# DocF/multispectral-object-detection

Hardware: AMD Instinct MI355X
Metric: image-pairs/sec fwd, yolov5l+CFTx3 640×640 bs64, 1/2/4/8 GPU (higher is better)
Workload: dtype bf16; 1 GPU; cfg3 (yolov5l_fusion_transformerx3_FLIR_aligned) two-stream forward, 640x640, 64 pairs/GPU, BN folded, pre-NMS detections; pairs_per_gpu=64, image_size=640, parallelism=batch-shard x1, hip_graph=True, two_hip_streams=False, forwards_in_flight=3, streams_per_forward_in_flight=1, single_in_flight_streams=2

## Files before the change

### include/cft_hip.h

```cpp
#ifndef CFT_HIP_H
#define CFT_HIP_H

#ifdef __cplusplus
extern "C" {
#endif

#define CFT_ABI_VERSION 19

enum { CFT_BF16 = 0, CFT_F32 = 1, CFT_F16 = 2 };
enum { CFT_ACT_NONE = 0, CFT_ACT_SILU = 1, CFT_ACT_GELU = 2 };
enum {
  CFT_OK = 0,
  CFT_EINVAL = -1,
  CFT_ELAUNCH = -2,
  CFT_ENODEV = -3
};

int cft_abi_version(void);
int cft_device_check(void);
const char* cft_last_error(void);
int cft_clock_probe(void* out4_u64, int spin_us, int* wall_khz, void* stream);

int cft_conv2d(const void* x, const void* w, const float* bias, const void* res, void* y,
               int B, int H, int W, int cin, int ldx, int xoff,
               int n, int kpad, int ksize, int stride,
               int ldy, int yoff, int ldr, int roff,
               int act, int dtype, int out_dtype, int res_dtype, void* stream);

int cft_conv2d_chain(const void* x, const void* w1, const float* bias1, const void* w2, const float* bias2, void* y,
                     int B, int H, int W, int cin, int ldx, int xoff,
                     int n1, int kpad1, int ksize, int stride, int n2,
                     int ldy, int yoff, int act2, int dtype, void* stream);
int cft_conv2d_chain_ok(int B, int H, int W, int cin, int ldx, int n1, int kpad1, int ksize, int stride, int n2, int ldy, int dtype);

int cft_conv2d_chain_res(const void* x, const void* w1, const float* bias1, const void* res, void* y1,
                         const void* w2, const float* bias2, void* y2,
                         int B, int H, int W, int cin, int ldx, int xoff,
                         int n1, int kpad1, int ksize, int stride, int ldr, int roff, int ldy1, int yoff1,
                         int n2, int ldy2, int yoff2, int act2, int dtype, void* stream);

int cft_linear_splitk(const void* x, const void* w, const float* bias, float* parts,
                      int rows, int cin, int ldx, int n, int kpad, int splits, int dtype, void* stream);

int cft_bottleneck(const void* x, int ldx, int xoff, const void* w1, int kpad1, const float* b1,
                   const void* w2, int kpad2, const void* w2_stages, const float* b2, void* y, int ldy, int yoff,
                   int B, int H, int W, int c, int shortcut, int dtype, void* stream);

int cft_bottleneck_pack_w2(const void* w2, int kpad2, int c, void* w2_stages, int dtype, void* stream);

int cft_set_conv_variant(int variant);

int cft_focus_s2d(const float* in, void* out, int B, int H, int W, int dtype, void* stream);

int cft_focus_s2d_u8(const unsigned char* in, long stride_b, long stride_c, long stride_h, void* out,
                     int B, int H, int W, float scale, int dtype, void* stream);

int cft_focus_conv(const void* in, int in_kind, long stride_b, long stride_c, long stride_h, float scale,
                   const void* w, int kpad, const float* bias, void* y, int ldy, int yoff,
                   int B, int H, int W, int n, int act, int dtype, void* stream);

int cft_spp_maxpool(void* buf, int B, int H, int W, int C, int ld, int k1, int k2, int k3,
                    int dtype, void* stream);

int cft_copy_channels(const void* in, int ldi, int ioff, void* out, int ldo, int ooff,
                      int B, int Ho, int Wo, int C, int up, int dtype, void* stream);

int cft_to_nhwc(const void* in, int in_dtype, long stride_b, long stride_c, long stride_h, long stride_w,
                void* out, int ldo, int ooff, int B, int C, int cpad, int H, int W, int dtype, void* stream);

int cft_letterbox_u8(const unsigned char* src, int src_h, int src_w, long src_row_stride,
                     unsigned char* dst, int dst_h, int dst_w, long dst_stride_y, long dst_stride_x, long dst_stride_c, int flip_channels,
                     int resized_h, int resized_w, int top, int left, int color0, int color1, int color2, void* stream);

enum { CFT_PAIR_COPY = 0, CFT_PAIR_LINEAR = 1, CFT_PAIR_AREA = 2 };
#define CFT_PAIR_DESC_BYTES 64
#define CFT_PAIR_MAX_REDUCTION 4
typedef struct {
  const unsigned char* src_rgb;
  const unsigned char* src_ir;
  long stride_rgb, stride_ir;
  int h0, w0;
  int h, w;
  int top, left;
  int mode, flip;
} cft_pair_desc_t;
int cft_pair_batch_u8(const void* desc_dev, const void* desc_host, int B, unsigned char* dst, int dst_h, int dst_w, int color, void* stream);

enum { CFT_AUG_FLIPLR = 1, CFT_AUG_FLIPUD = 2 };
#define CFT_AUG_DESC_BYTES 400
#define CFT_AUG_TILE_BYTES 80
#define CFT_AUG_MAX_SIDE 16384
typedef struct {
  const unsigned char* src_rgb;
  const unsigned char* src_ir;
  long stride_rgb, stride_ir;
  int h0, w0;
  int h, w;
  int x1, y1, x2, y2;
  int padw, padh;
  int reserved[2];
} cft_aug_tile_t;
// ... 155 lines not shown
```

### multispectral-object-detection_amd/csrc/bneck_common.h

```cpp
#pragma once
#include "cft_common.h"

struct Bneck128Params {
  const unsigned char* x;
  const unsigned char* w1;
  const unsigned char* w2;
  const unsigned char* w2s;
  const float* b1;
  const float* b2;
  unsigned char* y;
  int ldx, xoff, ldy, yoff, kpad1, kpad2;
  int H, W, tiles_x, tiles_y, ntiles, shortcut;
};

int bneck128_asm_launch(const Bneck128Params& p, int dtype, hipStream_t stream);
```

### multispectral-object-detection_amd/csrc/bottleneck.hip

```cpp
#include "cft_common.h"
#include <stdlib.h>

#ifdef CFT_PROBES
extern thread_local int g_conv_variant;
#endif

__device__ __attribute__((aligned(16))) uint32_t cft_zero_page_b[4] = {0u, 0u, 0u, 0u};
typedef __attribute__((address_space(3))) void lds_void_t;
typedef const __attribute__((address_space(1))) void gbl_void_t;

#include "bneck_common.h"

template <typename T, int ABL = 0>
__global__ void __launch_bounds__(512, 4) bottleneck128c_kernel(const Bneck128Params p) {
  constexpr int C = 128, TH = 8, TW = 16, PW = TW + 2, PH = TH + 2, NPIX = PW * PH;
  constexpr int NRT = (NPIX + 15) / 16;
  constexpr int PLANE = NRT * 16 * 128;
  constexpr int SLOT = 8192;
  constexpr int SLD = 64 + 4;
  constexpr int RW = 2;
  constexpr int XS = (ABL & 4) ? 0 : 2 * RW;
  static_assert(PW == 18 && NRT == 12, "the mul-shift below divides by 18; 8 + 4 row tiles");
  extern __shared__ __attribute__((aligned(16))) unsigned char smem[];
  unsigned char* sT = smem;
// ... 206 lines not shown
#undef BNC_MMA
#undef BNC_FETCH_RS

    if constexpr (ABL & 4) {
#pragma unroll
      for (int i = 0; i < RW; ++i)
#pragma unroll
        for (int j = 0; j < 4; ++j) asm volatile("" ::"v"(acc[i][j]));
    } else {
      float b2v[4];
#pragma unroll
      for (int j = 0; j < 4; ++j) b2v[j] = sB[C + wnc * 64 + j * 16 + lrow];
      asm volatile("s_waitcnt lgkmcnt(0)" ::: "memory");
      __builtin_amdgcn_s_barrier();
      float* stage = reinterpret_cast<float*>(sT) + wave * (16 * SLD);
#pragma unroll
      for (int i = 0; i < RW; ++i) {
#pragma unroll
        for (int j = 0; j < 4; ++j)
#pragma unroll
          for (int e = 0; e < 4; ++e)
            stage[(lgrp * 4 + e) * SLD + j * 16 + lrow] = apply_act<(ABL & 512) ? CFT_ACT_NONE : CFT_ACT_SILU>(acc[i][j][e] + b2v[j]);
        __builtin_amdgcn_fence(__ATOMIC_RELEASE, "wavefront");
        __builtin_amdgcn_wave_barrier();
        __builtin_amdgcn_fence(__ATOMIC_ACQUIRE, "wavefront");
#pragma unroll
        for (int v = 0; v < 2; ++v) {
          const int it = lane + v * 64;
          const int row = it >> 3, col = (it & 7) * 8;
          const int x = x0 + row, y = y0 + wmr * RW + i;
          if (x < p.W && y < p.H) {
            const f32x4_t s0 = *reinterpret_cast<const f32x4_t*>(stage + row * SLD + col);
            const f32x4_t s1 = *reinterpret_cast<const f32x4_t*>(stage + row * SLD + col + 4);
            float o[8] = {s0[0], s0[1], s0[2], s0[3], s1[0], s1[1], s1[2], s1[3]};
            if (p.shortcut) {
              float rf[8];
              Elem<T>::unpack(rs[i][v], rf);
#pragma unroll
              for (int e = 0; e < 8; ++e) o[e] += rf[e];
            }
            *reinterpret_cast<gran_t*>(p.y + ((img_pix + (long)y * p.W + x) * p.ldy + p.yoff + wnc * 64 + col) * 2) = Elem<T>::pack(o);
          }
        }
        __builtin_amdgcn_fence(__ATOMIC_RELEASE, "wavefront");
        __builtin_amdgcn_wave_barrier();
        __builtin_amdgcn_fence(__ATOMIC_ACQUIRE, "wavefront");
      }
    }
  }
#undef BNC_STAGE
#undef BNC_SYNC
}

template <typename T, int ABL = 0>
__global__ void __launch_bounds__(512, 4) bottleneck64r_kernel(const Bneck128Params p) {
  constexpr int C = 64, TS = 16, PW = TS + 2, NPIX = PW * PW;
  constexpr int NRT = (NPIX + 15) / 16;
  constexpr int PATCH = NRT * 16 * 128;
  constexpr int SLOT = 8192;
  constexpr int SLD = 64 + 4;
  constexpr int RW = 2, RT1 = 3;
  static_assert(PW == 18, "the mul-shift below divides by 18");
  extern __shared__ __attribute__((aligned(16))) unsigned char smem[];
  unsigned char* sT = smem;
  unsigned char* sR = smem + PATCH;
  float* sB = reinterpret_cast<float*>(smem + NPIX * 128);

  const int tid = threadIdx.x, lane = tid & 63;
  const int wave = __builtin_amdgcn_readfirstlane(tid >> 6);
  const int lrow = lane & 15, lgrp = lane >> 4;
  const int tiles = p.tiles_x * p.tiles_y;
  const int nb_ = gridDim.x, bid_ = blockIdx.x;
  const int xq_ = nb_ >> 3, xr_ = nb_ & 7, xcd_ = bid_ & 7, xslot_ = bid_ >> 3;
  const int ltile = (xcd_ < xr_ ? xcd_ * (xq_ + 1) : xr_ * (xq_ + 1) + (xcd_ - xr_) * xq_) + xslot_;
  const int b = ltile / tiles, tt = ltile - b * tiles;
  const int ty = tt / p.tiles_x, tx = tt - ty * p.tiles_x;
  const int y0 = ty * TS, x0 = tx * TS;
  const long img_pix = (long)b * p.H * p.W;
  const uint32_t tl = (uint32_t)(uintptr_t)(lds_void_t*)sT;

  const int r1 = tid >> 3, g1 = (tid & 7) ^ (r1 & 7);
  const unsigned char* src1 = p.w1 + ((long)r1 * p.kpad1 + g1 * 8) * 2;
  const unsigned char* src2 = p.w2 + ((long)r1 * p.kpad2 + g1 * 8) * 2;
#define BNR_STAGE(s_)                                                                                    \
  {                                                                                                      \
    const int ss_ = (s_);                                                                                \
    const unsigned char* src_ = ss_ == 0 ? src1 : src2 + (long)(ss_ - 1) * 128;                          \
    if constexpr (!(ABL & 8))                                                                            \
      __builtin_amdgcn_global_load_lds((gbl_void_t*)src_, (lds_void_t*)(sR + (ss_ & 3) * SLOT + wave * 1024), 16, 0, 0); \
  }
#define BNR_SYNC(n_)                                                                                     \
  {                                                                                                      \
    __builtin_amdgcn_sched_barrier(0);                                                                   \
    __builtin_amdgcn_s_waitcnt((n_) | 0x70);                                    \
    __builtin_amdgcn_s_barrier();                                                                        \
    __builtin_amdgcn_sched_barrier(0);                                                                   \
  }
  const int fb = lrow * 128 + ((lgrp ^ (lrow & 7)) << 4);

  gran_t a1[RT1][2];
  uint32_t keep[RT1];
#pragma unroll
  for (int it = 0; it < RT1; ++it) {
    const int q = (wave + 8 * it) * 16 + lrow;
    const int py = (q * 3641) >> 16, px = q - py * PW;
    const int zy = min(max(y0 - 1 + py, 0), p.H - 1), zx = min(max(x0 - 1 + px, 0), p.W - 1);
    keep[it] = (q < NPIX && (unsigned)(y0 - 1 + py) < (unsigned)p.H && (unsigned)(x0 - 1 + px) < (unsigned)p.W) ? 0xffffffffu : 0u;
    const unsigned char* xp = p.x + ((img_pix + (long)zy * p.W + zx) * p.ldx + p.xoff + lgrp * 8) * 2;
#pragma unroll
    for (int ks = 0; ks < 2; ++ks) {
      gran_t t = {0u, 0u, 0u, 0u};
      if (wave + 8 * it < NRT) t = *reinterpret_cast<const gran_t*>(xp + ks * 64);
      a1[it][ks] = t;
    }
  }
  __builtin_amdgcn_sched_barrier(0);
  BNR_STAGE(0)
  BNR_STAGE(1)
  BNR_STAGE(2)
  __builtin_amdgcn_sched_barrier(0);
  {
    float bq = 0.0f;
    if (tid < C) { if (p.b1 != nullptr) bq = p.b1[tid]; }
    else if (tid < 2 * C) { if (p.b2 != nullptr) bq = p.b2[tid - C]; }
    if (tid < 2 * C) sB[tid] = bq;
  }
  BNR_SYNC(0)
#pragma unroll
  for (int it = 0; it < RT1; ++it)
#pragma unroll
    for (int ks = 0; ks < 2; ++ks) {
      a1[it][ks].x &= keep[it]; a1[it][ks].y &= keep[it]; a1[it][ks].z &= keep[it]; a1[it][ks].w &= keep[it];
    }

  {
    f32x4_t acc1[RT1][4];
#pragma unroll
    for (int it = 0; it < RT1; ++it)
#pragma unroll
      for (int j = 0; j < 4; ++j) acc1[it][j] = f32x4_t{0.f, 0.f, 0.f, 0.f};
    BNR_STAGE(3)
    gran_t wf[4][2];
#pragma unroll
    for (int j = 0; j < 4; ++j) {
      wf[j][0] = *reinterpret_cast<const gran_t*>(sR + j * 2048 + fb);
      wf[j][1] = *reinterpret_cast<const gran_t*>(sR + j * 2048 + (fb ^ 64));
    }
    if constexpr (!(ABL & 1)) {
#pragma unroll
      for (int it = 0; it < RT1; ++it)
        if (wave + 8 * it < NRT) {
#pragma unroll
          for (int ks = 0; ks < 2; ++ks)
#pragma unroll
            for (int j = 0; j < 4; ++j) acc1[it][j] = mma_granule<T>(wf[j][ks], a1[it][ks], acc1[it][j]);
        }
    }
    BNR_SYNC(2)
#pragma unroll
    for (int it = 0; it < RT1; ++it) {
      const int q = (wave + 8 * it) * 16 + lrow;
      if (wave + 8 * it < NRT && q < NPIX) {
#pragma unroll
        for (int j = 0; j < 4; ++j) {
          const int cc = j * 16 + lgrp * 4;
          const f32x4_t b1q = *reinterpret_cast<const f32x4_t*>(sB + cc);
          float v[4];
#pragma unroll
          for (int e = 0; e < 4; ++e) v[e] = (ABL & 1) ? 0.0f : apply_act<CFT_ACT_SILU>(acc1[it][j][e] + b1q[e]);
          uint2 w;
          w.x = Elem<T>::pack2(v[0], v[1]) & keep[it];
          w.y = Elem<T>::pack2(v[2], v[3]) & keep[it];
          const uint32_t ta = tl + q * 128 + ((((cc >> 3) ^ (q & 7)) << 4) | ((cc & 7) << 1));
          const unsigned long long wq = ((unsigned long long)w.y << 32) | w.x;
          asm volatile("ds_write_b64 %0, %1" ::"v"(ta), "v"(wq) : "memory");
        }
      }
// ... 12 lines not shown
  for (int i = 0; i < RW; ++i) af[1][i] = gran_t{0u, 0u, 0u, 0u};
#pragma unroll
  for (int j = 0; j < 4; ++j) bf[1][j] = gran_t{0u, 0u, 0u, 0u};
#define BNR_READ(slot_, ks_)                                                                             \
  {                                                                                                      \
    _Pragma("unroll") for (int i = 0; i < RW; ++i) {                                                     \
      const int q = qb + i * PW;                                                                         \
      af[ks_][i] = *reinterpret_cast<const gran_t*>(sT + q * 128 + ((((ks_) * 4 + lgrp) ^ (q & 7)) << 4)); \
    }                                                                                                    \
    _Pragma("unroll") for (int j = 0; j < 4; ++j)                                                        \
      bf[ks_][j] = *reinterpret_cast<const gran_t*>(sR + (slot_) * SLOT + j * 2048 + ((ks_) ? (fb ^ 64) : fb)); \
    __builtin_amdgcn_sched_barrier(0);                                                                   \
  }
#define BNR_MMA(set_)                                                                                    \
  {                                                                                                      \
    _Pragma("unroll") for (int i = 0; i < RW; ++i)                                                       \
      _Pragma("unroll") for (int j = 0; j < 4; ++j) {                                                    \
        if constexpr (ABL & 2) { asm volatile("" ::"v"(af[set_][i]), "v"(bf[set_][j])); }                \
        else acc[i][j] = mma_granule<T>(af[set_][i], bf[set_][j], acc[i][j]);                            \
      }                                                                                                  \
    __builtin_amdgcn_sched_barrier(0);                                                                   \
  }
#pragma unroll
  for (int tap = 0; tap < 9; ++tap) {
    const int kh = tap / 3, kw = tap - kh * 3;
    const int qb = (wave * RW + kh) * PW + kw + lrow;
    if (tap + 4 <= 9) BNR_STAGE(tap + 4)
    BNR_READ((1 + tap) & 3, 0)
    BNR_MMA(1)
    BNR_READ((1 + tap) & 3, 1)
    BNR_MMA(0)
    if (tap <= 5) { BNR_SYNC(2) }
    else if (tap == 6) { BNR_SYNC(1) }
    else if (tap == 7) { BNR_SYNC(0) }
  }
  BNR_MMA(1)
#undef BNR_READ
#undef BNR_MMA
#undef BNR_STAGE
#undef BNR_SYNC

  if constexpr (ABL & 4) {
#pragma unroll
    for (int i = 0; i < RW; ++i)
#pragma unroll
      for (int j = 0; j < 4; ++j) asm volatile("" ::"v"(acc[i][j]));
    return;
  }
  float b2v[4];
#pragma unroll
  for (int j = 0; j < 4; ++j) b2v[j] = sB[C + j * 16 + lrow];
  asm volatile("s_waitcnt lgkmcnt(0)" ::: "memory");
  __builtin_amdgcn_s_barrier();
  if (p.shortcut) {
    int lane_e;
    asm volatile("v_mbcnt_lo_u32_b32 %0, -1, 0\n\tv_mbcnt_hi_u32_b32 %0, -1, %0" : "=v"(lane_e));
    const int lrow_e = lane_e & 15, lgrp_e = lane_e >> 4;
#pragma unroll
    for (int it = 0; it < RT1; ++it) {
      const int q = (wave + 8 * it) * 16 + lrow_e;
      const int py = (q * 3641) >> 16, px = q - py * PW;
      if (wave + 8 * it < NRT && py >= 1 && py <= TS && px >= 1 && px <= TS) {
        const int c = (py - 1) * TS + (px - 1);
#pragma unroll
        for (int ks = 0; ks < 2; ++ks)
          *reinterpret_cast<gran_t*>(sR + c * 128 + (((ks * 4 + lgrp_e) ^ (c & 7)) << 4)) = a1[it][ks];
      }
    }
    asm volatile("s_waitcnt lgkmcnt(0)" ::: "memory");
    __builtin_amdgcn_s_barrier();
  }
  float* stage = reinterpret_cast<float*>(sT) + wave * (16 * SLD);
#pragma unroll
  for (int i = 0; i < RW; ++i) {
#pragma unroll
    for (int j = 0; j < 4; ++j)
#pragma unroll
      for (int e = 0; e < 4; ++e)
        stage[(lgrp * 4 + e) * SLD + j * 16 + lrow] = apply_act<CFT_ACT_SILU>(acc[i][j][e] + b2v[j]);
    __builtin_amdgcn_fence(__ATOMIC_RELEASE, "wavefront");
    __builtin_amdgcn_wave_barrier();
    __builtin_amdgcn_fence(__ATOMIC_ACQUIRE, "wavefront");
#pragma unroll
    for (int v = 0; v < 2; ++v) {
      const int it = lane + v * 64;
      const int row = it >> 3, col = (it & 7) * 8;
      const int x = x0 + row, y = y0 + wave * RW + i;
      if (x < p.W && y < p.H) {
        const f32x4_t s0 = *reinterpret_cast<const f32x4_t*>(stage + row * SLD + col);
        const f32x4_t s1 = *reinterpret_cast<const f32x4_t*>(stage + row * SLD + col + 4);
        float o[8] = {s0[0], s0[1], s0[2], s0[3], s1[0], s1[1], s1[2], s1[3]};
        if (p.shortcut) {
          const int c = (wave * RW + i) * TS + row;
          const gran_t rsv = *reinterpret_cast<const gran_t*>(sR + c * 128 + (((it & 7) ^ (c & 7)) << 4));
          float rf[8];
          Elem<T>::unpack(rsv, rf);
#pragma unroll
          for (int e = 0; e < 8; ++e) o[e] += rf[e];
        }
        *reinterpret_cast<gran_t*>(p.y + ((img_pix + (long)y * p.W + x) * p.ldy + p.yoff + col) * 2) = Elem<T>::pack(o);
      }
    }
    __builtin_amdgcn_fence(__ATOMIC_RELEASE, "wavefront");
    __builtin_amdgcn_wave_barrier();
    __builtin_amdgcn_fence(__ATOMIC_ACQUIRE, "wavefront");
  }
}

__global__ void __launch_bounds__(256) bneck_pack_w2_kernel(const gran_t* __restrict__ w2, int kpad2, gran_t* __restrict__ out, int total) {
  const int i = blockIdx.x * 256 + threadIdx.x;
  if (i >= total) return;
  const int slot = i & 3, n = (i >> 2) & 127, u = i >> 9;
  const int kg = slot ^ ((0x1320 >> (4 * ((n >> 2) & 3))) & 3);
  out[i] = w2[(long)n * (kpad2 / 8) + u * 4 + kg];
}

extern "C" int cft_bottleneck_pack_w2(const void* w2, int kpad2, int c, void* w2_stages, int dtype, void* stream) {
  CFT_REQUIRE(w2 && w2_stages, "cft_bottleneck_pack_w2: null pointer");
  CFT_REQUIRE(dtype == CFT_BF16 || dtype == CFT_F16, "cft_bottleneck_pack_w2: dtype must be CFT_BF16 or CFT_F16");
  CFT_REQUIRE(c == 128 && kpad2 == 9 * 128, "cft_bottleneck_pack_w2: 128 channels, kpad2 = 1152");
  const int total = 36 * 128 * 4;
  hipLaunchKernelGGL(bneck_pack_w2_kernel, dim3((total + 255) / 256), dim3(256), 0, as_stream(stream),
                     (const gran_t*)w2, kpad2, (gran_t*)w2_stages, total);
// ... 27 lines not shown
  q.b1 = b1; q.b2 = b2; q.y = (unsigned char*)y;
  q.ldx = ldx; q.xoff = xoff; q.ldy = ldy; q.yoff = yoff; q.kpad1 = kpad1; q.kpad2 = kpad2;
  q.H = H; q.W = W; q.shortcut = shortcut ? 1 : 0;
  q.tiles_x = (W + 15) / 16; q.tiles_y = c == 128 ? (H + 7) / 8 : (H + 15) / 16;
  CFT_REQUIRE((long)B * q.tiles_x * q.tiles_y < (1L << 31), "cft_bottleneck: too many tiles");
  q.ntiles = B * q.tiles_x * q.tiles_y;
  hipStream_t s_ = as_stream(stream);
  const dim3 grid(q.ntiles);
#define BNC_LAUNCH(T_, ABL_)                                                                          \
  {                                                                                                   \
    constexpr int smem_ = 2 * 12 * 16 * 128 + 2 * 16384;                                              \
    cft_allow_lds<&bottleneck128c_kernel<T_, ABL_>>(smem_);                                           \
    hipLaunchKernelGGL((bottleneck128c_kernel<T_, ABL_>), grid, dim3(512), smem_, s_, q);             \
  }
#define BNR_LAUNCH(T_, ABL_)                                                                          \
  {                                                                                                   \
    constexpr int smem_ = 21 * 16 * 128 + 4 * 8192;                                                   \
    cft_allow_lds<&bottleneck64r_kernel<T_, ABL_>>(smem_);                                            \
    hipLaunchKernelGGL((bottleneck64r_kernel<T_, ABL_>), grid, dim3(512), smem_, s_, q);              \
  }
#ifdef CFT_PROBES
  if (dtype == CFT_BF16) {
    switch (g_conv_variant) {
      case 9201: if (c == 128) { BNC_LAUNCH(uint16_t, 1) return cft_check_launch("bottleneck128c_kernel(probe)"); } break;
      case 9202: if (c == 128) { BNC_LAUNCH(uint16_t, 2) return cft_check_launch("bottleneck128c_kernel(probe)"); } break;
      case 9204: if (c == 128) { BNC_LAUNCH(uint16_t, 4) return cft_check_launch("bottleneck128c_kernel(probe)"); } break;
      case 9208: if (c == 128) { BNC_LAUNCH(uint16_t, 8) return cft_check_launch("bottleneck128c_kernel(probe)"); } break;
      case 9456: if (c == 128) { BNC_LAUNCH(uint16_t, 256) return cft_check_launch("bottleneck128c_kernel(probe)"); } break;
      case 9712: if (c == 128) { BNC_LAUNCH(uint16_t, 512) return cft_check_launch("bottleneck128c_kernel(probe)"); } break;
      case 9601: if (c == 64) { BNR_LAUNCH(uint16_t, 1) return cft_check_launch("bottleneck64r_kernel(probe)"); } break;
      case 9602: if (c == 64) { BNR_LAUNCH(uint16_t, 2) return cft_check_launch("bottleneck64r_kernel(probe)"); } break;
      case 9604: if (c == 64) { BNR_LAUNCH(uint16_t, 4) return cft_check_launch("bottleneck64r_kernel(probe)"); } break;
      case 9608: if (c == 64) { BNR_LAUNCH(uint16_t, 8) return cft_check_launch("bottleneck64r_kernel(probe)"); } break;
      default: break;
    }
  }
#endif
  if (c == 128) {
#ifdef CFT_PROBES
    if (g_conv_variant == 98 || (g_conv_variant >= 9300 && g_conv_variant < 9400)) {
      q.tiles_y = (H + 15) / 16;
      q.ntiles = B * q.tiles_x * q.tiles_y;
      return bneck128_asm_launch(q, dtype, s_);
    }
#endif
    if (dtype == CFT_F16) BNC_LAUNCH(f16_t, 0) else BNC_LAUNCH(uint16_t, 0)
    return cft_check_launch("bottleneck128c_kernel");
  }
  if (dtype == CFT_F16) BNR_LAUNCH(f16_t, 0) else BNR_LAUNCH(uint16_t, 0)
#undef BNC_LAUNCH
#undef BNR_LAUNCH
  return cft_check_launch("bottleneck64r_kernel");
}
```

### multispectral-object-detection_amd/models/common.py

```python
import math
from collections import namedtuple

import torch
import torch.nn as nn

from .. import ops
from ..ops import ACT_GELU, ACT_NONE, ACT_SILU

BN_EPS = 1e-3


def autopad(k, p=None):
    if p is None:
        p = k // 2 if isinstance(k, int) else [x // 2 for x in k]
    return p


class _Pending:

    def materialize(self):
        raise NotImplementedError


class PendingBilinear(_Pending):
# ... 4 lines not shown
    def materialize(self, base=None):
        return ops.gpt_upsample_add(self.tokens, self.s, base, self.H, self.W, self.dtype, grid=self.grid)

    @property
    def shape(self):
        return torch.Size((self.tokens.shape[0], self.tokens.shape[2], self.H, self.W))


class PendingUpsample(_Pending):

    def __init__(self, x, up):
        self.x, self.up = x, up

    def materialize(self):
        B, C, H, W = self.x.shape
        out = ops.new_nhwc(B, H << self.up, W << self.up, C, self.x.dtype, self.x.device)
        return ops.copy_channels(self.x, out, self.up)

    @property
    def shape(self):
        B, C, H, W = self.x.shape
        return torch.Size((B, C, H << self.up, W << self.up))


class PendingConv(_Pending):

    def __init__(self, conv, x):
        self.conv, self.x = conv, x

    def materialize(self):
        return self.conv(self.x)

    @property
    def shape(self):
        B, _, H, W = self.x.shape
        return torch.Size((B, self.conv.conv.out_channels, *ops.conv_out_size(H, W, self.conv.conv.kernel_size[0], self.conv.conv.stride[0])))


def resolve(x):
    return x.materialize() if isinstance(x, _Pending) else x


def _cache_key(module, dtype, device):
    vers = tuple((int(p.data_ptr()), int(p._version)) for p in module.parameters()) \
        + tuple((int(b.data_ptr()), int(b._version)) for b in module.buffers())
    return (dtype, str(device), vers)


def invalidate_packed(root):
    for m in root.modules():
        m.__dict__.pop("_cft_cache", None)
        m.__dict__.pop("_cft_cache_train", None)
        m.__dict__.pop("_plan_cache", None)
        if "_graphs" in m.__dict__:
            m.__dict__["_graphs"].clear()
        m.__dict__.pop("_wlist", None)


class _Packed(nn.Module):

    def _packed(self, dtype, device, train=False):
        key = (train,) + _cache_key(self, dtype, device)
        slot = "_cft_cache_train" if train else "_cft_cache"
        cache = self.__dict__.get(slot)
        if cache is None or cache[0] != key:
            with torch.no_grad():
                cache = (key, self._pack_train(dtype, device) if train else self._pack(dtype, device))
            self.__dict__[slot] = cache
        return cache[1]

    def _pack_train(self, dtype, device):
        raise NotImplementedError(f"{type(self).__name__} has no training-mode form")

    def _pack(self, dtype, device):
        raise NotImplementedError


def _folded(conv_module):
    conv = conv_module.conv
    if hasattr(conv_module, "bn"):
        bn = conv_module.bn
        return ops.fold_bn(conv.weight, bn.weight, bn.bias, bn.running_mean, bn.running_var, bn.eps)
    bias = conv.bias.float() if conv.bias is not None else torch.zeros(conv.out_channels, device=conv.weight.device)
    return conv.weight.float(), bias


def _f32(t, device):
    return t.detach().to(device=device, dtype=torch.float32).contiguous()


def _act_code(act):
    if isinstance(act, nn.SiLU):
        return ACT_SILU
    if isinstance(act, nn.Identity):
        return ACT_NONE
    raise NotImplementedError(f"activation {type(act).__name__} has no fused epilogue (SiLU / Identity only)")


class Conv(_Packed):

    def __init__(self, c1, c2, k=1, s=1, p=None, g=1, act=True):
        super().__init__()
        if g != 1:
            raise NotImplementedError("grouped convolution is not used by any CFT config")
        if autopad(k, p) != k // 2:
            raise NotImplementedError("only 'same' padding (k//2) is implemented")
# ... 52 lines not shown
        self.cv1 = Conv(c1, c_, 1, 1)
        self.cv2 = Conv(c1, c_, 1, 1)
        self.cv3 = Conv(2 * c_, c2, 1)
        self.m = nn.Sequential(*[Bottleneck(c_, c_, shortcut, g, e=1.0) for _ in range(n)])

    def _pack(self, dtype, device):
        w1, b1 = _folded(self.cv1)
        w2, b2 = _folded(self.cv2)
        return ops.pack_conv(torch.cat([w1, w2], 0), torch.cat([b1, b2], 0), dtype, device=device)

    chain = True
    chain_pairs = True

    def launch_plan(self, B, H, W, dtype, front=None, ld_in=None):
        key = (front, B, H, W, ld_in, dtype, self.training, self.chain, self.chain_pairs, ops.CHAIN_RES_MIN_ROWS)
        cache = self.__dict__.setdefault("_plan_cache", {})
        if key not in cache:
            if len(cache) > 16:
                cache.clear()
            cache[key] = self._plan(B, H, W, dtype, front, ld_in)
        return cache[key]

    def _plan(self, B, H, W, dtype, front, ld_in):
        n = len(self.m)
        blocks = tuple(("block", j) for j in range(n))
        if self.training:
            return C3Plan(None if front is None else "separate", True, blocks)
        dev = self.cv1.conv.weight.device
        how = None
        if front is not None:
            ok = _act_code(front.act) == ACT_SILU and ops.conv2d_chain_ok_geometry(B, H, W, dtype, front._packed(dtype, dev), self._packed(dtype, dev), ldx=ld_in)
            how = "chained" if ok else "separate"
            H, W = ops.conv_out_size(H, W, front.conv.kernel_size[0], front.conv.stride[0])
        if not (self.chain and self.chain_pairs and n >= 2 and dtype in (torch.bfloat16, torch.float16)):
            return C3Plan(how, False, blocks)
        pks = [(b.cv1._packed(dtype, dev), b.cv2._packed(dtype, dev)) for b in self.m]
        acts = [(_act_code(b.cv1.act), _act_code(b.cv2.act)) for b in self.m]
        y = torch.empty((B, self.cv1.conv.out_channels, H, W), dtype=dtype, device="meta")
        own = [ops.bottleneck_fusable(y, *pk, *act) for pk, act in zip(pks, acts)]
        if (all(b.add for b in self.m) and all(a == (ACT_SILU, ACT_SILU) for a in acts) and not any(own)
                and all(ops.conv2d_chain_res_ok_geometry(B, H, W, dtype, pks[j][1], pks[j + 1][0]) for j in range(n - 1))):
            return C3Plan(how, False, (("cv1", 0),) + tuple(("pair_res", j) for j in range(n - 1)) + (("cv2", n - 1),))
        can = [j + 1 < n and not (self.m[j].add or self.m[j + 1].add or own[j]) and acts[j][1] == ACT_SILU
               and ops.conv2d_chain_ok_geometry(B, H, W, dtype, pks[j][1], pks[j + 1][0]) for j in range(n)]
        steps = []
        for j in range(n):
            entered = j > 0 and can[j - 1]
            if entered or can[j]:
                steps += ([] if entered else [("cv1", j)]) + [("pair" if can[j] else "cv2", j)]
            else:
                steps.append(("block", j))
        return C3Plan(how, False, tuple(steps))

    def forward(self, x, out=None):
        c_ = self.cv1.conv.out_channels
        act = _act_code(self.cv1.act)
        if act != _act_code(self.cv2.act):
            raise NotImplementedError("C3.cv1 and C3.cv2 must share an activation")
        front = x.conv if isinstance(x, PendingConv) else None
        x = resolve(x.x if front is not None else x)
        B, _, H, W = x.shape
        dt, dev = x.dtype, x.device
        plan = self.launch_plan(B, H, W, dt, front, x.stride(3) if (x.stride(1) == 1 and x.stride(3) >= x.shape[1]) else None)
        if plan.front == "chained":
            cat = ops.conv2d_chain(x, front._packed(dt, dev), self._packed(dt, dev), act)
        else:
            if front is not None:
                x = front(x)
            if plan.split:
                B, _, H, W = x.shape
                cat = ops.new_nhwc(B, H, W, 2 * c_, dt, dev)
                self.cv1(x, out=cat[:, :c_])
                self.cv2(x, out=cat[:, c_:])
            else:
                cat = ops.conv2d(x, self._packed(dt, dev), act)
        head = cat[:, :c_]
        y, h, last = head, None, len(self.m) - 1
        for form, j in plan.steps:
            blk, dst = self.m[j], (head if j == last else None)
            if form == "block":
                y = blk(y, out=dst)
            elif form == "cv1":
                h = blk.cv1(y)
            elif form == "cv2":
                y = blk.cv2(h, residual=y if blk.add else None, out=dst)
            else:
                nxt = self.m[j + 1].cv1
                pk2, pk1, act1 = blk.cv2._packed(dt, dev), nxt._packed(dt, dev), _act_code(nxt.act)
                if form == "pair":
                    h = ops.conv2d_chain(h, pk2, pk1, act1)
                else:
                    y, h = ops.conv2d_chain_res(h, pk2, y, pk1, act1)
        return self.cv3(cat, out=out)


class SPP(nn.Module):

    def __init__(self, c1, c2, k=(5, 9, 13)):
        super().__init__()
        c_ = c1 // 2
        self.cv1 = Conv(c1, c_, 1, 1)
        self.cv2 = Conv(c_ * (len(k) + 1), c2, 1, 1)
        self.m = nn.ModuleList([nn.MaxPool2d(kernel_size=x, stride=1, padding=x // 2) for x in k])
        self.k = tuple(k)

    def forward(self, x):
        x = resolve(x)
        ks = tuple(int(mp.kernel_size) for mp in self.m)
        if len(ks) != 3 or list(ks) != sorted(ks):
            raise NotImplementedError("SPP kernel implements exactly three ascending pooling sizes")
        c_ = self.cv1.conv.out_channels
        B, _, H, W = x.shape
        cat = ops.new_nhwc(B, H, W, 4 * c_, x.dtype, x.device)
        self.cv1(x, out=cat[:, :c_])
        ops.spp_maxpool(cat, c_, ks)
        return self.cv2(cat)


class Focus(_Packed):

    compute_dtype = None

    def __init__(self, c1, c2, k=1, s=1, p=None, g=1, act=True):
        super().__init__()
        self.conv = Conv(c1 * 4, c2, k, s, p, g, act)
        self.conv.cin_pad = 16

    def _pack(self, dtype, device):
        if self.conv.conv.in_channels != 12:
            raise NotImplementedError("Focus kernel is specialised for 3-channel images")
        return self.conv._pack(dtype, device, cin_pad=16)

# ... 450 lines not shown
```

### multispectral-object-detection_amd/ops.py

```python
from dataclasses import dataclass
from typing import Optional

import torch

from . import _lib
from ._lib import ACT_GELU, ACT_NONE, ACT_SILU, CFT_BF16, CFT_F16, CFT_F32


COMPUTE_DTYPES = (torch.bfloat16, torch.float16, torch.float32)


def _dt(dtype):
    if dtype == torch.bfloat16:
        return CFT_BF16
    if dtype == torch.float16:
        return CFT_F16
    if dtype == torch.float32:
        return CFT_F32
    raise TypeError(f"compute dtype must be torch.bfloat16, torch.float16 or torch.float32, got {dtype}")


def _stream():
    return torch.cuda.current_stream().cuda_stream

# ... 218 lines not shown
        out1 = new_nhwc(B, Ho, Wo, pk1.n, x.dtype, x.device)
    if out2 is None:
        out2 = new_nhwc(B, Ho, Wo, pk2.n, x.dtype, x.device)
    if tuple(out1.shape) != (B, pk1.n, Ho, Wo) or tuple(out2.shape) != (B, pk2.n, Ho, Wo) or out1.dtype != x.dtype or out2.dtype != x.dtype:
        raise ValueError("conv2d_chain_res: output shape / dtype mismatch")
    ldy1, ldy2 = _view_ld(out1, "conv2d_chain_res out1"), _view_ld(out2, "conv2d_chain_res out2")
    lib = _lib.load()
    es = x.element_size()
    M = B * Ho * Wo
    abytes = (B * H * W * pk1.cin + 2 * M * pk1.n_valid + M * pk2.n_valid + pk1.w.numel() + pk2.w.numel()) * es
    args = (x.data_ptr(), pk1.w.data_ptr(), _bias_ptr(pk1), res.data_ptr(), out1.data_ptr(), pk2.w.data_ptr(), _bias_ptr(pk2), out2.data_ptr(),
            B, H, W, pk1.cin, ldx, 0, pk1.n, pk1.kpad, pk1.k, pk1.s, ldr, 0, ldy1, 0, pk2.n, ldy2, 0, act2, _dt(x.dtype), _stream())
    st = _timed(f"conv_chainres_k{pk1.k}s{pk1.s}_n{pk1.n}_K{pk1.kpad}+{pk2.kpad}", M * (pk1.flops_per_row + pk2.flops_per_row), abytes,
                lambda: lib.cft_conv2d_chain_res(*args))
    _lib.check(st, "cft_conv2d_chain_res")
    return out1, out2


FUSED_BOTTLENECK_WIDTHS = (64, 128)


def bottleneck_fusable(x, pk1, pk2, act1, act2):
    return bottleneck_kernel_covers(x, pk1, pk2, act1, act2) and x.shape[1] in FUSED_BOTTLENECK_WIDTHS


def bottleneck_kernel_covers(x, pk1, pk2, act1, act2):
    return (x.dtype in (torch.bfloat16, torch.float16) and act1 == ACT_SILU and act2 == ACT_SILU
            and pk1.k == 1 and pk1.s == 1 and pk2.k == 3 and pk2.s == 1
            and pk1.cin == pk1.n == pk2.cin == pk2.n == x.shape[1] and x.shape[1] in (64, 128))


def bottleneck(x, pk1, pk2, shortcut, out=None):
    _require_cuda(x, "bottleneck")
    x, ldx = as_nhwc(x)
    B, C, H, W = x.shape
    if out is None:
        out = new_nhwc(B, H, W, C, x.dtype, x.device)
    if tuple(out.shape) != (B, C, H, W):
        raise ValueError(f"bottleneck: out has shape {tuple(out.shape)}, expected {(B, C, H, W)}")
    ldy = _view_ld(out, "bottleneck out")
    lib = _lib.load()
    if C == 128 and pk2.w_stages is None:
        pk2.w_stages = torch.empty_like(pk2.w)
        _lib.check(lib.cft_bottleneck_pack_w2(pk2.w.data_ptr(), pk2.kpad, C, pk2.w_stages.data_ptr(), _dt(x.dtype), _stream()),
                   "cft_bottleneck_pack_w2")
    args = (x.data_ptr(), ldx, 0, pk1.w.data_ptr(), pk1.kpad, _bias_ptr(pk1),
            pk2.w.data_ptr(), pk2.kpad, None if pk2.w_stages is None else pk2.w_stages.data_ptr(), _bias_ptr(pk2),
            out.data_ptr(), ldy, 0, B, H, W, C, 1 if shortcut else 0, _dt(x.dtype), _stream())
    rows = B * H * W
    abytes = rows * C * 2 * (3 if shortcut else 2) + (pk1.w.numel() + pk2.w.numel()) * 2
    st = _timed(f"conv_bneck_c{C}_K{pk1.kpad}+{pk2.kpad}", rows * (pk1.flops_per_row + pk2.flops_per_row), abytes,
                lambda: lib.cft_bottleneck(*args))
    _lib.check(st, "cft_bottleneck")
    return out


def linear(x, pk, act=ACT_NONE, residual=None, out=None, out_dtype=None):
    _require_cuda(x, "linear")
    rows, K = x.shape
    if K != pk.cin or x.stride(1) != 1:
        raise ValueError(f"linear: input [{rows},{K}] does not match packed weight (cin {pk.cin})")
    if out is None:
        out = torch.empty((rows, pk.n), dtype=out_dtype or x.dtype, device=x.device)
    rp, ldr, rdt = None, 0, CFT_BF16
    if residual is not None:
        rp, ldr, rdt = residual.data_ptr(), residual.stride(0), _dt(residual.dtype)
    lib = _lib.load()
    abytes = (rows * K * x.element_size() + rows * pk.n_valid * out.element_size() + pk.w.numel() * x.element_size()
              + (0 if residual is None else rows * pk.n_valid * residual.element_size()))
    st = _timed(f"linear_k{pk.k}s{pk.s}_n{pk.n}_K{pk.kpad}", rows * pk.flops_per_row, abytes,
                lambda: lib.cft_conv2d(x.data_ptr(), pk.w.data_ptr(), _bias_ptr(pk), rp, out.data_ptr(), 1, 1, rows, pk.cin, x.stride(0), 0,
                                       pk.n, pk.kpad, 1, 1, out.stride(0), 0, ldr, 0, act, _dt(x.dtype), _dt(out.dtype), rdt, _stream()))
    _lib.check(st, "cft_conv2d(linear)")
    return out


SPLITK_MAX_ROWS = 1024


def splitk_choice(rows, pk, dtype):
    bk = 32 if dtype == torch.float32 else 64
    if pk.k != 1 or pk.kpad != pk.cin or pk.cin % bk or 2 * pk.kpad * (4 if dtype == torch.float32 else 2) + 128 > 65536:
        return 1
    steps = pk.kpad // bk
    t256 = -(-rows // 256) * -(-pk.n // 256)
    if t256 >= 64 or rows > SPLITK_MAX_ROWS:
        return 1
    best = 1
    for s in (2, 4, 8):
        if steps % s or steps // s < 4 or s * rows * pk.n >= 2 ** 31:
            break
        best = s
        if t256 * s >= 128:
            break
    return best


def linear_splitk(x, pk, splits):
    _require_cuda(x, "linear_splitk")
    rows, K = x.shape
    if K != pk.cin or x.stride(1) != 1:
        raise ValueError(f"linear_splitk: input [{rows},{K}] does not match packed weight (cin {pk.cin})")
    parts = torch.empty((splits, rows, pk.n), dtype=torch.float32, device=x.device)
    lib = _lib.load()
    abytes = rows * K * x.element_size() + splits * rows * pk.n_valid * 4 + pk.w.numel() * x.element_size()
    st = _timed(f"linear_k{pk.k}s{pk.s}_n{pk.n}_K{pk.kpad}", rows * pk.flops_per_row, abytes,
# ... 506 lines not shown
```

Measured before the change: 3618 image-pairs/sec.

## Fuse C3 cv3 1x1 conv into the last 64-channel bottleneck kernel

Adds a TAIL variant of the 64-channel bottleneck kernel. It keeps the bottleneck output in LDS, loads the matching cv2 half of the concat, and computes the cv3 1x1 conv (128->128) with SiLU directly, writing the C3 output. The goal is to avoid writing the bottleneck result to global memory, re-reading the concat, and paying a separate cv3 launch. In exchange the kernel does extra LDS staging, more barriers and more register use, and adds the eligibility and overlap checks needed to route C3 blocks onto the fused path.

After: 3637 image-pairs/sec, median of 6. Within noise of the previous version (+0.5%).

```diff
diff --git a/include/cft_hip.h b/include/cft_hip.h
--- a/include/cft_hip.h
+++ b/include/cft_hip.h
@@ -47,6 +47,12 @@
                    int B, int H, int W, int c, int shortcut, int dtype, void* stream);
 
 int cft_bottleneck_pack_w2(const void* w2, int kpad2, int c, void* w2_stages, int dtype, void* stream);
+
+int cft_bottleneck_cv3(const void* x, int ldx, int xoff, const void* w1, int kpad1, const float* b1,
+                       const void* w2, int kpad2, const void* w2_stages, const float* b2,
+                       const void* c2, int ldc, int coff, const void* w3, int kpad3, const void* w3_stages, const float* b3,
+                       void* out, int ldo, int ooff, int B, int H, int W, int c, int shortcut, int dtype, void* stream);
+int cft_bottleneck_cv3_ok(int B, int H, int W, int c, int ldx, int ldc, int ldo, int dtype);
 
 int cft_set_conv_variant(int variant);
 
diff --git a/multispectral-object-detection_amd/csrc/bneck_common.h b/multispectral-object-detection_amd/csrc/bneck_common.h
--- a/multispectral-object-detection_amd/csrc/bneck_common.h
+++ b/multispectral-object-detection_amd/csrc/bneck_common.h
@@ -11,6 +11,10 @@
   unsigned char* y;
   int ldx, xoff, ldy, yoff, kpad1, kpad2;
   int H, W, tiles_x, tiles_y, ntiles, shortcut;
+  const unsigned char* c2;
+  const unsigned char* w3;
+  const float* b3;
+  int ldc, coff, kpad3;
 };
 
 int bneck128_asm_launch(const Bneck128Params& p, int dtype, hipStream_t stream);
diff --git a/multispectral-object-detection_amd/csrc/bottleneck.hip b/multispectral-object-detection_amd/csrc/bottleneck.hip
--- a/multispectral-object-detection_amd/csrc/bottleneck.hip
+++ b/multispectral-object-detection_amd/csrc/bottleneck.hip
@@ -282,7 +282,7 @@
 #undef BNC_SYNC
 }
 
-template <typename T, int ABL = 0>
+template <typename T, int ABL = 0, bool TAIL = false>
 __global__ void __launch_bounds__(512, 4) bottleneck64r_kernel(const Bneck128Params p) {
   constexpr int C = 64, TS = 16, PW = TS + 2, NPIX = PW * PW;
   constexpr int NRT = (NPIX + 15) / 16;
@@ -353,6 +353,10 @@
     float bq = 0.0f;
     if (tid < C) { if (p.b1 != nullptr) bq = p.b1[tid]; }
     else if (tid < 2 * C) { if (p.b2 != nullptr) bq = p.b2[tid - C]; }
+    if constexpr (TAIL) {
+      if (tid >= 2 * C && tid < 4 * C && p.b3 != nullptr) bq = p.b3[tid - 2 * C];
+      if (tid >= 2 * C && tid < 4 * C) reinterpret_cast<float*>(sR + 4 * SLOT)[tid - 2 * C] = bq;
+    }
     if (tid < 2 * C) sB[tid] = bq;
   }
   BNR_SYNC(0)
@@ -471,6 +475,29 @@
   for (int j = 0; j < 4; ++j) b2v[j] = sB[C + j * 16 + lrow];
   asm volatile("s_waitcnt lgkmcnt(0)" ::: "memory");
   __builtin_amdgcn_s_barrier();
+  constexpr int HLD = 32 + 4;
+  [[maybe_unused]] unsigned char* sW = sT + 8 * 16 * HLD * 4;
+  [[maybe_unused]] gran_t cf[RW][2];
+  if constexpr (TAIL) {
+    int lane_t;
+    asm volatile("v_mbcnt_lo_u32_b32 %0, -1, 0\n\tv_mbcnt_hi_u32_b32 %0, -1, %0" : "=v"(lane_t));
+#pragma unroll
+    for (int i = 0; i < RW; ++i) {
+      const int yy = min(y0 + wave * RW + i, p.H - 1), xx = min(x0 + (lane_t & 15), p.W - 1);
+      const unsigned char* cp = p.c2 + ((img_pix + (long)yy * p.W + xx) * p.ldc + p.coff + (lane_t >> 4) * 8) * 2;
+#pragma unroll
+      for (int ks = 0; ks < 2; ++ks) cf[i][ks] = *reinterpret_cast<const gran_t*>(cp + ks * 64);
+    }
+    __builtin_amdgcn_sched_barrier(0);
+    const int tid_t = wave * 64 + lane_t;
+    const int r3 = tid_t >> 3, g3 = (tid_t & 7) ^ (r3 & 7);
+    const unsigned char* src3 = p.w3 + ((long)r3 * p.kpad3 + g3 * 8) * 2;
+#pragma unroll
+    for (int u = 0; u < 3; ++u)
+      __builtin_amdgcn_global_load_lds((gbl_void_t*)(src3 + ((long)(u >> 1) * 64 * p.kpad3 + (u & 1) * 64) * 2),
+                                       (lds_void_t*)(sW + u * SLOT + wave * 1024), 16, 0, 0);
+    __builtin_amdgcn_sched_barrier(0);
+  }
   if (p.shortcut) {
     int lane_e;
     asm volatile("v_mbcnt_lo_u32_b32 %0, -1, 0\n\tv_mbcnt_hi_u32_b32 %0, -1, %0" : "=v"(lane_e));
@@ -482,12 +509,129 @@
       if (wave + 8 * it < NRT && py >= 1 && py <= TS && px >= 1 && px <= TS) {
         const int c = (py - 1) * TS + (px - 1);
 #pragma unroll
-        for (int ks = 0; ks < 2; ++ks)
-          *reinterpret_cast<gran_t*>(sR + c * 128 + (((ks * 4 + lgrp_e) ^ (c & 7)) << 4)) = a1[it][ks];
+        for (int ks = 0; ks < 2; ++ks) {
+          if constexpr (TAIL)
+            asm volatile("ds_write_b128 %0, %1" ::"v"(tl + PATCH + c * 128 + (((ks * 4 + lgrp_e) ^ (c & 7)) << 4)), "v"(a1[it][ks]) : "memory");
+          else
+            *reinterpret_cast<gran_t*>(sR + c * 128 + (((ks * 4 + lgrp_e) ^ (c & 7)) << 4)) = a1[it][ks];
+        }
       }
     }
     asm volatile("s_waitcnt lgkmcnt(0)" ::: "memory");
     __builtin_amdgcn_s_barrier();
+  }
+  if constexpr (TAIL) {
+    int lane_t;
+    asm volatile("v_mbcnt_lo_u32_b32 %0, -1, 0\n\tv_mbcnt_hi_u32_b32 %0, -1, %0" : "=v"(lane_t));
+    const int lrow_t = lane_t & 15, lgrp_t = lane_t >> 4;
+    const int row = lane_t >> 2, gq = lane_t & 3;
+    const uint32_t st_w = tl + wave * (16 * HLD * 4) + ((lgrp_t * 4) * HLD + lrow_t) * 4;
+    const float* st_r = reinterpret_cast<const float*>(sT) + wave * (16 * HLD) + row * HLD + gq * 8;
+#define BNT_STRIP(a_, bv_, hh_, o_)                                                                      \
+    {                                                                                                    \
+      _Pragma("unroll") for (int jj = 0; jj < 2; ++jj)                                                   \
+        _Pragma("unroll") for (int e = 0; e < 4; ++e) {                                                  \
+          const float v_ = apply_act<CFT_ACT_SILU>((a_)[2 * (hh_) + jj][e] + (bv_)[2 * (hh_) + jj]);     \
+          asm volatile("ds_write_b32 %0, %1 offset:%2" ::"v"(st_w), "v"(v_), "i"((e * HLD + jj * 16) * 4) : "memory"); \
+        }                                                                                                \
+      __builtin_amdgcn_fence(__ATOMIC_RELEASE, "wavefront");                                             \
+      __builtin_amdgcn_wave_barrier();                                                                   \
+      __builtin_amdgcn_fence(__ATOMIC_ACQUIRE, "wavefront");                                             \
+      const f32x4_t s0_ = *reinterpret_cast<const f32x4_t*>(st_r);                                       \
+      const f32x4_t s1_ = *reinterpret_cast<const f32x4_t*>(st_r + 4);                                   \
+      o_[0] = s0_[0]; o_[1] = s0_[1]; o_[2] = s0_[2]; o_[3] = s0_[3];                                    \
+      o_[4] = s1_[0]; o_[5] = s1_[1]; o_[6] = s1_[2]; o_[7] = s1_[3];                                    \
+      asm volatile("s_waitcnt lgkmcnt(0)" ::: "memory");   \
+      __builtin_amdgcn_fence(__ATOMIC_RELEASE, "wavefront");                                             \
+      __builtin_amdgcn_wave_barrier();                                                                   \
+      __builtin_amdgcn_fence(__ATOMIC_ACQUIRE, "wavefront");                                             \
+    }
+#pragma unroll
+    for (int i = 0; i < RW; ++i) {
+      const int c = (wave * RW + i) * TS + row;
+#pragma unroll
+      for (int hh = 0; hh < 2; ++hh) {
+        float o[8];
+        BNT_STRIP(acc[i], b2v, hh, o)
+        const int ya = c * 128 + (((hh * 4 + gq) ^ (c & 7)) << 4);
+        if (p.shortcut) {
+          const gran_t rsv = *reinterpret_cast<const gran_t*>(sR + ya);
+          float rf[8];
+          Elem<T>::unpack(rsv, rf);
+#pragma unroll
+          for (int e = 0; e < 8; ++e) o[e] += rf[e];
+        }
+        const gran_t yv = Elem<T>::pack(o);
+        asm volatile("ds_write_b128 %0, %1" ::"v"(tl + PATCH + ya), "v"(yv) : "memory");
+      }
+    }
+    __builtin_amdgcn_fence(__ATOMIC_RELEASE, "wavefront");
+    __builtin_amdgcn_wave_barrier();
+    __builtin_amdgcn_fence(__ATOMIC_ACQUIRE, "wavefront");
+    gran_t yf[RW][2];
+#pragma unroll
+    for (int i = 0; i < RW; ++i) {
+      const int c = (wave * RW + i) * TS + lrow_t;
+#pragma unroll
+      for (int ks = 0; ks < 2; ++ks) yf[i][ks] = *reinterpret_cast<const gran_t*>(sR + c * 128 + (((ks * 4 + lgrp_t) ^ (c & 7)) << 4));
+    }
+    __builtin_amdgcn_sched_barrier(0);
+    __builtin_amdgcn_s_waitcnt(0 | 0x70);
+    __builtin_amdgcn_s_barrier();
+    __builtin_amdgcn_sched_barrier(0);
+    {
+      const int tid_t = wave * 64 + lane_t;
+      const int r3 = tid_t >> 3, g3 = (tid_t & 7) ^ (r3 & 7);
+      __builtin_amdgcn_global_load_lds((gbl_void_t*)(p.w3 + ((long)(64 + r3) * p.kpad3 + 64 + g3 * 8) * 2),
+                                       (lds_void_t*)(sR + wave * 1024), 16, 0, 0);
+    }
+    __builtin_amdgcn_sched_barrier(0);
+    const int fb_t = lrow_t * 128 + ((lgrp_t ^ (lrow_t & 7)) << 4);
+    const float* sB3 = reinterpret_cast<const float*>(sR + 4 * SLOT);
+#pragma unroll
+    for (int nh = 0; nh < 2; ++nh) {
+      f32x4_t acc3[RW][4];
+#pragma unroll
+      for (int i = 0; i < RW; ++i)
+#pragma unroll
+        for (int j = 0; j < 4; ++j) acc3[i][j] = f32x4_t{0.f, 0.f, 0.f, 0.f};
+#pragma unroll
+      for (int kh = 0; kh < 2; ++kh) {
+        const unsigned char* wb = (nh * 2 + kh < 3) ? sW + (nh * 2 + kh) * SLOT : sR;
+#pragma unroll
+        for (int ks = 0; ks < 2; ++ks) {
+          gran_t bw[4];
+#pragma unroll
+          for (int j = 0; j < 4; ++j) bw[j] = *reinterpret_cast<const gran_t*>(wb + j * 2048 + (ks ? (fb_t ^ 64) : fb_t));
+#pragma unroll
+          for (int i = 0; i < RW; ++i)
+#pragma unroll
+            for (int j = 0; j < 4; ++j) acc3[i][j] = mma_granule<T>(kh == 0 ? yf[i][ks] : cf[i][ks], bw[j], acc3[i][j]);
+        }
+        if (nh == 0 && kh == 1) {
+          __builtin_amdgcn_sched_barrier(0);
+          __builtin_amdgcn_s_waitcnt(0 | 0x70);
+          __builtin_amdgcn_s_barrier();
+          __builtin_amdgcn_sched_barrier(0);
+        }
+      }
+      float b3v[4];
+#pragma unroll
+      for (int j = 0; j < 4; ++j) b3v[j] = sB3[nh * 64 + j * 16 + lrow_t];
+#pragma unroll
+      for (int i = 0; i < RW; ++i) {
+        const int x = x0 + row, y = y0 + wave * RW + i;
+#pragma unroll
+        for (int hh = 0; hh < 2; ++hh) {
+          float o[8];
+          BNT_STRIP(acc3[i], b3v, hh, o)
+          if (x < p.W && y < p.H)
+            *reinterpret_cast<gran_t*>(p.y + ((img_pix + (long)y * p.W + x) * p.ldy + p.yoff + nh * 64 + hh * 32 + gq * 8) * 2) = Elem<T>::pack(o);
+        }
+      }
+    }
+#undef BNT_STRIP
+    return;
   }
   float* stage = reinterpret_cast<float*>(sT) + wave * (16 * SLD);
 #pragma unroll
@@ -621,3 +765,65 @@
 #undef BNR_LAUNCH
   return cft_check_launch("bottleneck64r_kernel");
 }
+
+static const char* bneck_cv3_refusal(int B, int H, int W, int c, int ldx, int ldc, int ldo, int dtype) {
+  if (dtype != CFT_BF16 && dtype != CFT_F16) return "cft_bottleneck_cv3: dtype must be CFT_BF16 or CFT_F16";
+  if (c != 64) return "cft_bottleneck_cv3: the tail kernel covers 64 channels (run cft_bottleneck and cft_conv2d otherwise)";
+  if (B <= 0 || H <= 0 || W <= 0) return "cft_bottleneck_cv3: non-positive size";
+  if (ldx % 8 != 0 || ldc % 8 != 0 || ldo % 8 != 0 || ldx < c || ldc < c || ldo < 2 * c) return "cft_bottleneck_cv3: ld must be a multiple of 8 and cover the channel slice";
+  const long pix = (long)B * H * W;
+  if (pix * ldx >= (1L << 31) || pix * ldc >= (1L << 31) || pix * ldo >= (1L << 31)) return "cft_bottleneck_cv3: tensor exceeds 2^31 elements";
+  if ((long)B * ((W + 15) / 16) * ((H + 15) / 16) >= (1L << 31)) return "cft_bottleneck_cv3: too many tiles";
+  return nullptr;
+}
+
+extern "C" int cft_bottleneck_cv3_ok(int B, int H, int W, int c, int ldx, int ldc, int ldo, int dtype) {
+  return bneck_cv3_refusal(B, H, W, c, ldx, ldc, ldo, dtype) == nullptr ? 1 : 0;
+}
+
+static bool bneck_slices_disjoint(const char* pa, long lda, int wa, const char* pb, long ldb, int wb, long pix) {
+  if (pa + ((pix - 1) * lda + wa) * 2 <= pb || pb + ((pix - 1) * ldb + wb) * 2 <= pa) return true;
+  if (lda != ldb) return false;
+  const long d = pb > pa ? pb - pa : pa - pb;
+  const int wlo = pb > pa ? wa : wb, whi = pb > pa ? wb : wa;
+  return d >= (long)wlo * 2 && d + (long)whi * 2 <= lda * 2;
+}
+
+extern "C" int cft_bottleneck_cv3(const void* x, int ldx, int xoff, const void* w1, int kpad1, const float* b1,
+                                  const void* w2, int kpad2, const void* w2_stages, const float* b2,
+                                  const void* c2, int ldc, int coff, const void* w3, int kpad3, const void* w3_stages, const float* b3,
+                                  void* out, int ldo, int ooff, int B, int H, int W, int c, int shortcut, int dtype, void* stream) {
+  (void)w2_stages; (void)w3_stages;
+  CFT_REQUIRE(x && w1 && w2 && c2 && w3 && out, "cft_bottleneck_cv3: null pointer");
+  const char* why = bneck_cv3_refusal(B, H, W, c, ldx, ldc, ldo, dtype);
+  CFT_REQUIRE(why == nullptr, why);
+  CFT_REQUIRE(kpad1 >= c && kpad1 % 64 == 0 && kpad2 >= 9 * c && kpad2 % 64 == 0 && kpad3 >= 2 * c && kpad3 % 64 == 0,
+              "cft_bottleneck_cv3: weights must be packed as for cft_conv2d");
+  CFT_REQUIRE(xoff % 8 == 0 && coff % 8 == 0 && ooff % 8 == 0 && xoff >= 0 && coff >= 0 && ooff >= 0 && ldx >= xoff + c && ldc >= coff + c && ldo >= ooff + 2 * c,
+              "cft_bottleneck_cv3: offsets must be multiples of 8 and the slices must fit their pixels");
+  {
+    const long pix = (long)B * H * W;
+    const char* xa = (const char*)x + (long)xoff * 2;
+    const char* ca = (const char*)c2 + (long)coff * 2;
+    const char* oa = (const char*)out + (long)ooff * 2;
+    CFT_REQUIRE(bneck_slices_disjoint(xa, ldx, c, oa, ldo, 2 * c, pix) && bneck_slices_disjoint(ca, ldc, c, oa, ldo, 2 * c, pix),
+                "cft_bottleneck_cv3: output overlaps x or the cv2 half");
+  }
+  Bneck128Params q;
+  q.x = (const unsigned char*)x; q.w1 = (const unsigned char*)w1; q.w2 = (const unsigned char*)w2; q.w2s = nullptr;
+  q.b1 = b1; q.b2 = b2; q.y = (unsigned char*)out;
+  q.ldx = ldx; q.xoff = xoff; q.ldy = ldo; q.yoff = ooff; q.kpad1 = kpad1; q.kpad2 = kpad2;
+  q.H = H; q.W = W; q.shortcut = shortcut ? 1 : 0;
+  q.tiles_x = (W + 15) / 16; q.tiles_y = (H + 15) / 16;
+  q.ntiles = B * q.tiles_x * q.tiles_y;
+  q.c2 = (const unsigned char*)c2; q.w3 = (const unsigned char*)w3; q.b3 = b3; q.ldc = ldc; q.coff = coff; q.kpad3 = kpad3;
+  constexpr int smem = 21 * 16 * 128 + 4 * 8192 + 128 * 4;
+  if (dtype == CFT_F16) {
+    cft_allow_lds<&bottleneck64r_kernel<f16_t, 0, true>>(smem);
+    hipLaunchKernelGGL((bottleneck64r_kernel<f16_t, 0, true>), dim3(q.ntiles), dim3(512), smem, as_stream(stream), q);
+  } else {
+    cft_allow_lds<&bottleneck64r_kernel<uint16_t, 0, true>>(smem);
+    hipLaunchKernelGGL((bottleneck64r_kernel<uint16_t, 0, true>), dim3(q.ntiles), dim3(512), smem, as_stream(stream), q);
+  }
+  return cft_check_launch("bottleneck64r_kernel(tail)");
+}
diff --git a/multispectral-object-detection_amd/models/common.py b/multispectral-object-detection_amd/models/common.py
--- a/multispectral-object-detection_amd/models/common.py
+++ b/multispectral-object-detection_amd/models/common.py
@@ -80,6 +80,7 @@
         m.__dict__.pop("_cft_cache", None)
         m.__dict__.pop("_cft_cache_train", None)
         m.__dict__.pop("_plan_cache", None)
+        m.__dict__.pop("_tail_cache", None)
         if "_graphs" in m.__dict__:
             m.__dict__["_graphs"].clear()
         m.__dict__.pop("_wlist", None)
@@ -238,6 +239,32 @@
                 steps.append(("block", j))
         return C3Plan(how, False, tuple(steps))
 
+    fuse_tail = True
+
+    def tail_fused(self, B, H, W, dtype, ld_out=None):
+        key = (B, H, W, dtype, ld_out, self.training, self.fuse_tail, self.chain, self.chain_pairs, ops.CHAIN_RES_MIN_ROWS, type(self.cv3.act))
+        cache = self.__dict__.setdefault("_tail_cache", {})
+        if key not in cache:
+            if len(cache) > 16:
+                cache.clear()
+            cache[key] = self._tail(B, H, W, dtype, ld_out)
+        return cache[key]
+
+    def _tail(self, B, H, W, dtype, ld_out):
+        n, c_ = len(self.m), self.cv1.conv.out_channels
+        if not self.fuse_tail or self.training or n == 0 or dtype not in (torch.bfloat16, torch.float16):
+            return False
+        if not isinstance(self.cv3.act, nn.SiLU) or self.cv3.conv.out_channels != 2 * c_ or self.cv3.conv.in_channels != 2 * c_:
+            return False
+        steps = self._plan(B, H, W, dtype, None, None).steps
+        if not steps or steps[-1] != ("block", n - 1):
+            return False
+        dev, blk = self.cv1.conv.weight.device, self.m[n - 1]
+        y = torch.empty((B, c_, H, W), dtype=dtype, device="meta")
+        if not ops.bottleneck_fusable(y, blk.cv1._packed(dtype, dev), blk.cv2._packed(dtype, dev), _act_code(blk.cv1.act), _act_code(blk.cv2.act)):
+            return False
+        return ops.bottleneck_cv3_ok_geometry(B, H, W, dtype, c_, ld_out=ld_out)
+
     def forward(self, x, out=None):
         c_ = self.cv1.conv.out_channels
         act = _act_code(self.cv1.act)
@@ -262,8 +289,12 @@
                 cat = ops.conv2d(x, self._packed(dt, dev), act)
         head = cat[:, :c_]
         y, h, last = head, None, len(self.m) - 1
+        tail = self.tail_fused(cat.shape[0], cat.shape[2], cat.shape[3], dt, None if out is None else out.stride(3))
         for form, j in plan.steps:
             blk, dst = self.m[j], (head if j == last else None)
+            if tail and form == "block" and j == last:
+                return ops.bottleneck_cv3(y, blk.cv1._packed(dt, dev), blk.cv2._packed(dt, dev), blk.add, cat[:, c_:],
+                                          self.cv3._packed(dt, dev), out=out)
             if form == "block":
                 y = blk(y, out=dst)
             elif form == "cv1":
diff --git a/multispectral-object-detection_amd/ops.py b/multispectral-object-detection_amd/ops.py
--- a/multispectral-object-detection_amd/ops.py
+++ b/multispectral-object-detection_amd/ops.py
@@ -294,6 +294,53 @@
     st = _timed(f"conv_bneck_c{C}_K{pk1.kpad}+{pk2.kpad}", rows * (pk1.flops_per_row + pk2.flops_per_row), abytes,
                 lambda: lib.cft_bottleneck(*args))
     _lib.check(st, "cft_bottleneck")
+    return out
+
+
+def bottleneck_cv3_ok_geometry(B, H, W, dtype, c, ld_out=None, ldx=None, ldc=None):
+    if dtype not in (torch.bfloat16, torch.float16):
+        return False
+    return bool(_lib.load().cft_bottleneck_cv3_ok(B, H, W, c, ldx or 2 * c, ldc or 2 * c, ld_out or 2 * c, _dt(dtype)))
+
+
+def _slices_disjoint(a, lda, b, ldb):
+    es = a.element_size()
+    pix = a.shape[0] * a.shape[2] * a.shape[3]
+    pa, pb = a.data_ptr(), b.data_ptr()
+    if pa + ((pix - 1) * lda + a.shape[1]) * es <= pb or pb + ((pix - 1) * ldb + b.shape[1]) * es <= pa:
+        return True
+    if lda != ldb:
+        return False
+    (lo, wlo), (hi, whi) = sorted(((pa, a.shape[1]), (pb, b.shape[1])))
+    return hi - lo >= wlo * es and hi - lo + whi * es <= lda * es
+
+
+def bottleneck_cv3(x, pk1, pk2, shortcut, c2, pk3, out=None):
+    _require_cuda(x, "bottleneck_cv3")
+    B, C, H, W = x.shape
+    if not bottleneck_kernel_covers(x, pk1, pk2, ACT_SILU, ACT_SILU):
+        raise ValueError("bottleneck_cv3: not a Bottleneck cft_bottleneck implements (bottleneck_kernel_covers)")
+    if tuple(c2.shape) != (B, C, H, W) or c2.dtype != x.dtype or pk3.cin != 2 * C or pk3.k != 1 or pk3.s != 1 or pk3.n != 2 * C:
+        raise ValueError(f"bottleneck_cv3: x {tuple(x.shape)}, c2 {tuple(c2.shape)} and a {pk3.cin} -> {pk3.n} cv3 do not form a C3 tail")
+    ldx, ldc = _view_ld(x, "bottleneck_cv3 x"), _view_ld(c2, "bottleneck_cv3 c2")
+    if out is None:
+        out = new_nhwc(B, H, W, pk3.n, x.dtype, x.device)
+    if tuple(out.shape) != (B, pk3.n, H, W) or out.dtype != x.dtype:
+        raise ValueError(f"bottleneck_cv3: out has shape {tuple(out.shape)}, expected {(B, pk3.n, H, W)}")
+    ldo = _view_ld(out, "bottleneck_cv3 out")
+    if not (_slices_disjoint(x, ldx, out, ldo) and _slices_disjoint(c2, ldc, out, ldo)):
+        raise ValueError("bottleneck_cv3: out overlaps x or c2")
+    if not bottleneck_cv3_ok_geometry(B, H, W, x.dtype, C, ld_out=ldo, ldx=ldx, ldc=ldc):
+        raise ValueError("bottleneck_cv3: shape not eligible (bottleneck_cv3_ok_geometry)")
+    lib = _lib.load()
+    args = (x.data_ptr(), ldx, 0, pk1.w.data_ptr(), pk1.kpad, _bias_ptr(pk1), pk2.w.data_ptr(), pk2.kpad, None, _bias_ptr(pk2),
+            c2.data_ptr(), ldc, 0, pk3.w.data_ptr(), pk3.kpad, None, _bias_ptr(pk3),
+            out.data_ptr(), ldo, 0, B, H, W, C, 1 if shortcut else 0, _dt(x.dtype), _stream())
+    rows = B * H * W
+    abytes = rows * (2 * C + pk3.n_valid) * 2 + (pk1.w.numel() + pk2.w.numel() + pk3.w.numel()) * 2
+    st = _timed(f"conv_bnecktail_c{C}_K{pk1.kpad}+{pk2.kpad}+{pk3.kpad}", rows * (pk1.flops_per_row + pk2.flops_per_row + pk3.flops_per_row), abytes,
+                lambda: lib.cft_bottleneck_cv3(*args))
+    _lib.check(st, "cft_bottleneck_cv3")
     return out
 
 
```
